# speedinghzl/CCNet

Hardware: NVIDIA H100
Metric: cca_fwd_bwd_pixels_per_s (higher is better)
Workload: dtype f32

## Files before the change

ccnet_b200/csrc/cca_tc_bwd.cuh:

```cuda
#pragma once
#include "cca_items.cuh"
#include "cca_tc_common.cuh"

namespace cca {
namespace tc {

struct BwdParams {
    ItemSpace sp;
    int C, Cq;
    long npix;
    const float *lse;
    float *delta;
    unsigned int *ddone;
    int delta_mode;
    int out_mode;
    unsigned int *cdone;
    int lag;
    int hints;
};

template <int LK, typename E> struct BwdSmem {
    using T = Tiles<LK, E>;
    static constexpr int kCh = T::H16 ? kNC : kNC / 2;
    static constexpr int kRSlot = T::kTile;
    static constexpr int off_qk = 0;
    static constexpr int off_p = off_qk + 2 * T::kSlot;
    static constexpr int off_ld = (off_p + T::kP + (16 - LK / 8) * T::kPlane + 1023) / 1024 * 1024;
    static constexpr int kTail = (128 - LK) * 128 + 256;
    static constexpr int kDsum = 1024;
    static constexpr int kBudget = 232448;
    static constexpr int kNLd = (kBudget - off_ld - kTail - kDsum - 16) / (kRSlot + 16);
    static constexpr int off_tail = off_ld + kNLd * kRSlot;
    static constexpr int off_dsum = off_tail + kTail;
    static constexpr int off_bar = off_dsum + kDsum;
    static constexpr int kBytes = off_bar + 8 * (2 + 2 * kNLd);
    static_assert(kNLd >= 8, "ring depth: chunk n - 1's dO (staged dV) up to chunk n + 1's O");
    static_assert(off_p % 1024 == 0 && T::kP >= T::kSlot, "dK staging in the P / dS planes");
    static_assert(kBytes <= kBudget, "shared memory budget");
};

__device__ __forceinline__ bool calc_delta(const BwdParams &p, const Item &it) { return p.delta_mode == 0 || (it.col && it.ik == 0); }

template <int LK, typename E>
__global__ void __launch_bounds__(kThreads, 1)
cca_tc_bwd_kernel(const __grid_constant__ CUtensorMap mqc, const __grid_constant__ CUtensorMap mqr,
                  const __grid_constant__ CUtensorMap mkc, const __grid_constant__ CUtensorMap mkr,
                  const __grid_constant__ CUtensorMap mvc, const __grid_constant__ CUtensorMap mvr,
                  const __grid_constant__ CUtensorMap mdoc, const __grid_constant__ CUtensorMap mdor,
                  const __grid_constant__ CUtensorMap moc, const __grid_constant__ CUtensorMap mor,
                  const __grid_constant__ CUtensorMap mdqc, const __grid_constant__ CUtensorMap mdqr,
                  const __grid_constant__ CUtensorMap mdkc, const __grid_constant__ CUtensorMap mdkr,
                  const __grid_constant__ CUtensorMap mdvc, const __grid_constant__ CUtensorMap mdvr, BwdParams p)
{
    using T = Tiles<LK, E>;
    using S = BwdSmem<LK, E>;
    constexpr bool H16 = kH16<E>, F16 = kF16<E>;
    constexpr int TERMS = H16 ? 1 : 3;
    constexpr int kNLd = S::kNLd;
    constexpr int kCh = S::kCh;
    constexpr int KP = LK / 16;
    constexpr uint32_t LOP = T::kPP * T::kPlane;
    extern __shared__ __align__(1024) uint8_t smem[];
    uint64_t *bars = reinterpret_cast<uint64_t *>(smem + S::off_bar);
    uint64_t *qk_full = bars, *qk_empty = bars + 1, *full = bars + 2, *empty = bars + 2 + kNLd;
    float *dsum = reinterpret_cast<float *>(smem + S::off_dsum);
    const int tid = threadIdx.x, warp = tid >> 5, lane = tid & 31;
    const int NCH = p.C / kCh;
    const int KQ = p.Cq / 16;
    const int nk = p.sp.total > (int)blockIdx.x ? (p.sp.total - (int)blockIdx.x + (int)gridDim.x - 1) / (int)gridDim.x : 0;
    auto item_of = [&](int k) { return decode_item_order(p.sp, (int)blockIdx.x + k * (int)gridDim.x, p.lag); };

    if (tid == 0) {
        mbar_init(qk_full, 1); mbar_init(qk_empty, 1);
        for (int i = 0; i < kNLd; ++i) { mbar_init(&full[i], 1); mbar_init(&empty[i], 1); }
        fence_mbar_init();
        prefetch_tmap(&mqc); prefetch_tmap(&mqr); prefetch_tmap(&mkc); prefetch_tmap(&mkr); prefetch_tmap(&mvc); prefetch_tmap(&mvr);
        prefetch_tmap(&mdoc); prefetch_tmap(&mdor); prefetch_tmap(&moc); prefetch_tmap(&mor);
        prefetch_tmap(&mdqc); prefetch_tmap(&mdqr); prefetch_tmap(&mdkc); prefetch_tmap(&mdkr); prefetch_tmap(&mdvc); prefetch_tmap(&mdvr);
    }
    __syncthreads();

    if (tid < 128) {
        setmaxnreg_dec<kProducerRegs>();
        if (warp == 0 && lane == 0) {
            const uint64_t pol_keep = l2_policy_evict_last(), pol_stream = l2_policy_evict_first();
            auto load = [&](uint8_t *dst, uint64_t *bar, const CUtensorMap *m, int c0, const Item &it, int start, bool last_use, int boxes) {
                const int cw = it.col ? it.line : start, ch = it.col ? start : it.line;
                if (p.hints == 1) {
                    const uint64_t pol = (is_producer(it) && !last_use) ? pol_keep : pol_stream;
                    for (int bx = 0; bx < boxes; ++bx) tma_load_4d(dst + bx * T::kTile, m, bar, c0 + 32 * bx, cw, ch, it.b, pol);
                } else {
                    for (int bx = 0; bx < boxes; ++bx) tma_load_4d(dst + bx * T::kTile, m, bar, c0 + 32 * bx, cw, ch, it.b);
                }
            };
            uint32_t g = 0;
            auto ring = [&](const CUtensorMap *m, int c0, const Item &it, int start, bool last_use) {
                const int slot = g % kNLd;
                mbar_wait(&empty[slot], ((g / kNLd) & 1) ^ 1);
                mbar_expect_tx(&full[slot], S::kRSlot);
                load(smem + S::off_ld + slot * S::kRSlot, &full[slot], m, c0, it, start, last_use, 1);
                ++g;
            };
            for (int k = 0; k < nk; ++k) {
                const Item it = item_of(k);
                const bool calc = calc_delta(p, it);
                mbar_wait(qk_empty, (k & 1) ^ 1);
                mbar_expect_tx(qk_full, 2 * T::kSlot);
                load(smem + S::off_qk, qk_full, it.col ? &mqc : &mqr, 0, it, it.q0, false, H16 ? 1 : 2);
                load(smem + S::off_qk + T::kSlot, qk_full, it.col ? &mkc : &mkr, 0, it, it.k0, false, H16 ? 1 : 2);
                for (int n = 0; n < NCH; ++n) {
                    ring(it.col ? &mvc : &mvr, n * kCh, it, it.k0, false);
                    ring(it.col ? &mdoc : &mdor, n * kCh, it, it.q0, false);
                    if (calc) ring(it.col ? &moc : &mor, n * kCh, it, it.q0, p.delta_mode == 1);
                }
            }
        }
    } else {
        setmaxnreg_inc<kConsumerRegs>();
        const int t = tid - 128, wg = t >> 7, wq = (t >> 5) & 3;
        const int rbase = 64 * wg + 16 * wq + (lane >> 2);
        const int cq = 2 * (lane & 3);
        const uint32_t qb = smem_u32(smem + S::off_qk), kb = qb + T::kSlot, ld_base = smem_u32(smem + S::off_ld);
        const uint32_t pb = smem_u32(smem + S::off_p);
        uint8_t *pgen = smem + S::off_p;
        const uint64_t pol_keep = l2_policy_evict_last(), pol_stream = l2_policy_evict_first();
        auto stage = [&](const float *acc, int nc, uint8_t *tile) {
#pragma unroll
            for (int h = 0; h < 2; ++h) {
                const int r = rbase + 8 * h;
                if (r >= LK) continue;
                uint8_t *row = tile + r * 128;
#pragma unroll
                for (int j = 0; j < 8; ++j) {
                    if (8 * j >= nc) break;
                    const int c = 8 * j + cq;
                    const int bx = H16 ? 0 : c >> 5, byte = H16 ? 2 * c : 4 * (c & 31);
                    uint8_t *dst = row + bx * T::kTile + ((((byte >> 4) ^ r) & 7) << 4) + (byte & 15);
                    if constexpr (H16) *reinterpret_cast<uint32_t *>(dst) = pack2<F16>(acc[4 * j + 2 * h], acc[4 * j + 2 * h + 1]);
                    else *reinterpret_cast<float2 *>(dst) = make_float2(acc[4 * j + 2 * h], acc[4 * j + 2 * h + 1]);
                }
            }
        };
        auto put = [&](const CUtensorMap *m, const uint8_t *tile, int boxes, int c0, int px0, const Item &it, bool prod) {
            const int cw = it.col ? it.line : px0, ch = it.col ? px0 : it.line;
            for (int bx = 0; bx < boxes; ++bx) {
                const uint8_t *src = tile + bx * T::kTile;
                if (p.hints == 1) {
                    if (prod) tma_store_4d(m, src, c0 + 32 * bx, cw, ch, it.b, pol_keep);
                    else tma_reduce_add_4d(m, src, c0 + 32 * bx, cw, ch, it.b, pol_stream);
                } else {
                    if (prod) tma_store_4d(m, src, c0 + 32 * bx, cw, ch, it.b);
                    else tma_reduce_add_4d(m, src, c0 + 32 * bx, cw, ch, it.b);
                }
            }
            bulk_commit();
        };
        const int qboxes = H16 ? 1 : (p.Cq > 32 ? 2 : 1);
        pdl_wait();
        uint32_t g = 0;
        int pending = -1;
        for (int k = 0; k < nk; ++k) {
            const Item it = item_of(k);
            const bool calc = calc_delta(p, it);
            const bool prod = p.out_mode == 1 && is_producer(it);
            long qpix[2];
            bool qok[2];
            float nlse[2];
            int self[2];
#pragma unroll
            for (int h = 0; h < 2; ++h) {
                const int r = rbase + 8 * h;
                qok[h] = r < it.lq;
                qpix[h] = item_pixel(p.sp, it, qok[h] ? r : 0);
                nlse[h] = qok[h] ? -p.lse[qpix[h]] * kLog2e : 0.f;
                self[h] = it.col ? it.q0 + r - it.k0 : -1;
            }
            mbar_wait(qk_full, k & 1);
            if constexpr (!H16) {
                convert_slot<LK, E>(smem + S::off_qk, t);
                convert_slot<LK, E>(smem + S::off_qk + T::kSlot, t);
            }
            {
                float acc[LK / 2];
                wg_fence();
                for (int ks = 0; ks < KQ; ++ks) {
                    wgmma_ss<LK, F16>(acc, desc_kmaj<LK, E>(qb, 64 * wg, ks, false), desc_kmaj<LK, E>(kb, 0, ks, false), ks > 0, 0, 0);
                    if constexpr (TERMS == 3) {
                        wgmma_ss<LK, F16>(acc, desc_kmaj<LK, E>(qb, 64 * wg, ks, false), desc_kmaj<LK, E>(kb, 0, ks, true), 1, 0, 0);
                        wgmma_ss<LK, F16>(acc, desc_kmaj<LK, E>(qb, 64 * wg, ks, true), desc_kmaj<LK, E>(kb, 0, ks, false), 1, 0, 0);
                    }
                }
                wg_commit();
                wg_wait<0>();
                wg_acc_fence<LK / 2>(acc);
                if (t == 0) bulk_wait_read<0>();
                consumers_sync();
#pragma unroll
                for (int j = 0; j < LK / 8; ++j)
#pragma unroll
                    for (int h = 0; h < 2; ++h) {
                        const int r = rbase + 8 * h, c = 8 * j + cq;
                        const bool ok0 = qok[h] && c < it.lk && c != self[h];
                        const bool ok1 = qok[h] && c + 1 < it.lk && c + 1 != self[h];
                        const float p0 = ok0 ? exp2f(fmaf(acc[4 * j + 2 * h], kLog2e, nlse[h])) : 0.f;
                        const float p1 = ok1 ? exp2f(fmaf(acc[4 * j + 2 * h + 1], kLog2e, nlse[h])) : 0.f;
                        if (r < LK) {
                            uint8_t *d = pgen + j * T::kPlane + r * 16 + cq * 2;
                            if constexpr (H16) {
                                *reinterpret_cast<uint32_t *>(d) = pack2<F16>(p0, p1);
                            } else {
                                uint32_t hi, lo;
                                split2(p0, p1, hi, lo);
                                *reinterpret_cast<uint32_t *>(d) = hi;
                                *reinterpret_cast<uint32_t *>(d + LOP) = lo;
                            }
                        }
                    }
            }
            fence_proxy_async();
            consumers_sync();
            if (!prod && p.out_mode == 1) wait_count(p.cdone + it.b, (unsigned)p.sp.seg0);
            if (!prod && t == 0) fence_proxy_async_global();
            float dp[LK / 2];
            float o[kCh / 2];
            float dacc = 0.f;
            const uint32_t per = calc ? 3 : 2;
            auto rslot = [&](uint32_t gi) { return gi % kNLd; };
            auto convert_chunk = [&](int n) {
                const uint32_t gv = g + per * n, gd = gv + 1, go = gv + 2;
                mbar_wait(&full[rslot(gv)], (gv / kNLd) & 1);
                mbar_wait(&full[rslot(gd)], (gd / kNLd) & 1);
                if (calc) mbar_wait(&full[rslot(go)], (go / kNLd) & 1);
                uint8_t *vs = smem + S::off_ld + rslot(gv) * S::kRSlot, *ds = smem + S::off_ld + rslot(gd) * S::kRSlot;
                if constexpr (!H16) convert_slot<LK, E, 1>(vs, t);
                if (calc) {
                    dacc += convert_slot<LK, E, 1>(ds, t, smem + S::off_ld + rslot(go) * S::kRSlot);
                    if constexpr (H16) consumers_sync();
                    if (t == 0) mbar_arrive(&empty[rslot(go)]);
                } else if constexpr (!H16) {
                    convert_slot<LK, E, 1>(ds, t);
                }
            };
            auto issue = [&](int n) {
                const uint32_t gv = g + per * n, gd = gv + 1;
                const uint32_t vb = ld_base + rslot(gv) * S::kRSlot, db = ld_base + rslot(gd) * S::kRSlot;
                wg_fence();
#pragma unroll
                for (int ks = 0; ks < kCh / 16; ++ks) {
                    wgmma_ss<LK, F16>(dp, desc_kmaj<LK, E>(db, 64 * wg, ks, false), desc_kmaj<LK, E>(vb, 0, ks, false), n > 0 || ks > 0, 0, 0);
                    if constexpr (TERMS == 3) {
                        wgmma_ss<LK, F16>(dp, desc_kmaj<LK, E>(db, 64 * wg, ks, false), desc_kmaj<LK, E>(vb, 0, ks, true), 1, 0, 0);
                        wgmma_ss<LK, F16>(dp, desc_kmaj<LK, E>(db, 64 * wg, ks, true), desc_kmaj<LK, E>(vb, 0, ks, false), 1, 0, 0);
                    }
                }
#pragma unroll
                for (int ks = 0; ks < KP; ++ks) {
                    const uint32_t pa = pb + 8 * wg * T::kPlane + ks * 256;
                    if constexpr (H16) {
                        wgmma_ss_n64<F16>(o, smem_desc(pa, 128, T::kPlane), desc_mnmaj<LK, E>(db, ks, false), ks > 0, 1, 1);
                    } else {
                        wgmma_ss_n32<1, 1>(o, smem_desc(pa, 128, T::kPlane), desc_mnmaj<LK, E>(db, ks, false), ks > 0);
                        wgmma_ss_n32<1, 1>(o, smem_desc(pa, 128, T::kPlane), desc_mnmaj<LK, E>(db, ks, true), 1);
                        wgmma_ss_n32<1, 1>(o, smem_desc(pa + LOP, 128, T::kPlane), desc_mnmaj<LK, E>(db, ks, false), 1);
                    }
                }
                wg_commit();
            };
            auto release = [&]() {
                if (t == 0 && pending >= 0) {
                    bulk_wait_read<0>();
                    mbar_arrive(&empty[pending]);
                    pending = -1;
                }
            };
            auto retire = [&](int n) {
                const uint32_t gv = g + per * n, gd = gv + 1;
                wg_acc_fence<kCh / 2>(o);
                consumers_sync();
                if (t == 0) mbar_arrive(&empty[rslot(gv)]);
                uint8_t *ds = smem + S::off_ld + rslot(gd) * S::kRSlot;
                stage(o, kCh, ds);
                fence_proxy_async();
                consumers_sync();
                if (t == 0) {
                    put(it.col ? &mdvc : &mdvr, ds, 1, n * kCh, it.k0, it, prod);
                    pending = (int)rslot(gd);
                }
            };
            convert_chunk(0);
            issue(0);
            for (int n = 0; n < NCH; ++n) {
                if (n + 1 < NCH) convert_chunk(n + 1);
                release();
                wg_wait<0>();
                retire(n);
                if (n + 1 < NCH) issue(n + 1);
            }
            wg_wait<0>();
            wg_acc_fence<LK / 2>(dp);
            g += per * NCH;
            float dl[2] = {0.f, 0.f};
            if (calc) {
                dsum[(t >> 7) * 128 + (t & 127)] = dacc;
                consumers_sync();
#pragma unroll
                for (int h = 0; h < 2; ++h) {
                    const int r = rbase + 8 * h;
                    dl[h] = dsum[r] + dsum[128 + r];
                    if (qok[h] && is_producer(it) && (lane & 3) == 0) p.delta[qpix[h]] = dl[h];
                }
                if (p.delta_mode == 1) {
                    __threadfence();
                    consumers_sync();
                    if (t == 0) atomicAdd(p.ddone + it.b, 1u);
                }
            } else {
                wait_count(p.ddone + it.b, (unsigned)p.sp.seg0);
#pragma unroll
                for (int h = 0; h < 2; ++h) dl[h] = qok[h] ? __ldcg(p.delta + qpix[h]) : 0.f;
            }
            consumers_sync();
#pragma unroll
            for (int j = 0; j < LK / 8; ++j)
#pragma unroll
                for (int h = 0; h < 2; ++h) {
                    const int r = rbase + 8 * h;
                    if (r < LK) {
                        uint8_t *d = pgen + j * T::kPlane + r * 16 + cq * 2;
                        const uint32_t hw = *reinterpret_cast<const uint32_t *>(d);
                        const uint32_t lw = H16 ? 0u : *reinterpret_cast<const uint32_t *>(d + LOP);
                        const float p0 = lo2<F16>(hw) + lo2<F16>(lw), p1 = hi2<F16>(hw) + hi2<F16>(lw);
                        const float s0 = qok[h] ? p0 * (dp[4 * j + 2 * h] - dl[h]) : 0.f;
                        const float s1 = qok[h] ? p1 * (dp[4 * j + 2 * h + 1] - dl[h]) : 0.f;
                        if constexpr (H16) {
                            *reinterpret_cast<uint32_t *>(d) = pack2<F16>(s0, s1);
                        } else {
                            uint32_t hi, lo;
                            split2(s0, s1, hi, lo);
                            *reinterpret_cast<uint32_t *>(d) = hi;
                            *reinterpret_cast<uint32_t *>(d + LOP) = lo;
                        }
                    }
                }
            fence_proxy_async();
            consumers_sync();
            {
                float aq[32], ak[32];
                wg_fence();
#pragma unroll
                for (int ks = 0; ks < KP; ++ks) {
                    const uint32_t a = pb + 64 * wg * 16 + ks * 2 * T::kPlane;
                    wgmma_ss_n64<F16>(aq, smem_desc(a, T::kPlane, 128), desc_mnmaj<LK, E>(kb, ks, false), ks > 0, 0, 1);
                    if constexpr (TERMS == 3) {
                        wgmma_ss_n64<F16>(aq, smem_desc(a, T::kPlane, 128), desc_mnmaj<LK, E>(kb, ks, true), 1, 0, 1);
                        wgmma_ss_n64<F16>(aq, smem_desc(a + LOP, T::kPlane, 128), desc_mnmaj<LK, E>(kb, ks, false), 1, 0, 1);
                    }
                }
                wg_commit();
                wg_wait<0>();
                wg_acc_fence<32>(aq);
                consumers_sync();
                stage(aq, 64, smem + S::off_qk + T::kSlot);
                fence_proxy_async();
                consumers_sync();
                if (t == 0) put(it.col ? &mdqc : &mdqr, smem + S::off_qk + T::kSlot, qboxes, 0, it.q0, it, prod);
                wg_fence();
#pragma unroll
                for (int ks = 0; ks < KP; ++ks) {
                    const uint32_t at = pb + 8 * wg * T::kPlane + ks * 256;
                    wgmma_ss_n64<F16>(ak, smem_desc(at, 128, T::kPlane), desc_mnmaj<LK, E>(qb, ks, false), ks > 0, 1, 1);
                    if constexpr (TERMS == 3) {
                        wgmma_ss_n64<F16>(ak, smem_desc(at, 128, T::kPlane), desc_mnmaj<LK, E>(qb, ks, true), 1, 1, 1);
                        wgmma_ss_n64<F16>(ak, smem_desc(at + LOP, 128, T::kPlane), desc_mnmaj<LK, E>(qb, ks, false), 1, 1, 1);
                    }
                }
                wg_commit();
                wg_wait<0>();
                wg_acc_fence<32>(ak);
                consumers_sync();
                stage(ak, 64, pgen);
                fence_proxy_async();
                consumers_sync();
                if (t == 0) {
                    put(it.col ? &mdkc : &mdkr, pgen, qboxes, 0, it.k0, it, prod);
                    bulk_wait_read<1>();
                    if (pending >= 0) mbar_arrive(&empty[pending]);
                    pending = -1;
                    mbar_arrive(qk_empty);
                    if (prod) {
                        bulk_wait<0>();
                        publish_count(p.cdone + it.b);
                    }
                }
            }
        }
        if (t == 0) bulk_wait<0>();
    }
}

namespace {
__global__ void __launch_bounds__(256) cca_bwd_prep_kernel(uint4 *dq, uint4 *dk, uint4 *dv, long nq16, long nv16,
                                                           unsigned int *counters, int n_counters)
{
    pdl_launch_dependents();
    const long tid = (long)blockIdx.x * blockDim.x + threadIdx.x, nth = (long)gridDim.x * blockDim.x;
    const uint4 z = make_uint4(0, 0, 0, 0);
    for (long i = tid; i < nq16; i += nth) { dq[i] = z; dk[i] = z; }
    for (long i = tid; i < nv16; i += nth) dv[i] = z;
    for (long i = tid; i < n_counters; i += nth) counters[i] = 0u;
}
}

template <int LK, typename E>
cudaError_t launch_bwd(const void *dout, const void *q, const void *k, const void *v, const void *out, const float *lse, float *delta,
                       unsigned int *counters, void *dq, void *dk, void *dv, Dims d, int delta_mode, cudaStream_t st,
                       const char **why)
{
    CUtensorMap m[16];
    const void *base[8] = {q, k, v, dout, out, dq, dk, dv};
    const int ch[8] = {d.Cq, d.Cq, d.C, d.C, d.C, d.Cq, d.Cq, d.C};
    BwdParams p;
    p.sp = make_space(d.B, d.H, d.W);
    for (int t = 0; t < 8; ++t)
        for (int r = 0; r < 2; ++r) {
            const int box = t < 5 ? LK : (r == 0 ? p.sp.col.tl : p.sp.row.tl);
            if (!get_map(&m[2 * t + r], base[t], d.B, d.H, d.W, ch[t], box, r == 0, kDtype<E>)) {
                if (why) *why = "cuTensorMapEncodeTiled failed";
                return cudaErrorInvalidValue;
            }
        }
    p.C = d.C; p.Cq = d.Cq;
    p.npix = (long)d.B * d.H * d.W;
    p.lse = lse; p.delta = delta;
    p.ddone = counters; p.cdone = counters + d.B;
    p.delta_mode = delta_mode;
    const bool one_tile = p.sp.col.nt == 1 && p.sp.row.nt == 1;
    p.out_mode = one_tile ? 1 : 0;
    p.lag = tc_lag() != 0 ? 1 : 0;
    p.hints = tc_l2_hints();
    const long es = sizeof(E);
    const long nq = p.out_mode == 1 ? 0 : p.npix * d.Cq * es, nv = p.out_mode == 1 ? 0 : p.npix * d.C * es;
    cca_bwd_prep_kernel<<<p.out_mode == 1 ? 1 : sm_count(), 256, 0, st>>>(
        reinterpret_cast<uint4 *>(dq), reinterpret_cast<uint4 *>(dk), reinterpret_cast<uint4 *>(dv), nq / 16, nv / 16, counters, 3 * d.B);
    count_launch();
    cudaError_t e = cudaGetLastError();
    if (e != cudaSuccess) return e;
    auto kern = cca_tc_bwd_kernel<LK, E>;
    e = cudaFuncSetAttribute(kern, cudaFuncAttributeMaxDynamicSharedMemorySize, BwdSmem<LK, E>::kBytes);
    if (e != cudaSuccess) return e;
    const int sms = sm_count();
    const int grid = p.sp.total < sms ? p.sp.total : sms;
    cudaLaunchConfig_t cfg = {};
    cfg.gridDim = dim3(grid); cfg.blockDim = dim3(kThreads); cfg.dynamicSmemBytes = BwdSmem<LK, E>::kBytes; cfg.stream = st;
    cudaLaunchAttribute attr[1];
    attr[0].id = cudaLaunchAttributeProgrammaticStreamSerialization;
    attr[0].val.programmaticStreamSerializationAllowed = 1;
    cfg.attrs = attr;
    cfg.numAttrs = tc_pdl() ? 1 : 0;
    e = cudaLaunchKernelEx(&cfg, kern, m[0], m[1], m[2], m[3], m[4], m[5], m[6], m[7], m[8], m[9], m[10], m[11], m[12], m[13],
                           m[14], m[15], p);
    count_launch();
    return e != cudaSuccess ? e : cudaGetLastError();
}


extern template cudaError_t launch_bwd<80, __half>(const void *, const void *, const void *, const void *, const void *, const float *,
                                                   float *, unsigned int *, void *, void *, void *, Dims, int, cudaStream_t,
                                                   const char **);
extern template cudaError_t launch_bwd<112, __half>(const void *, const void *, const void *, const void *, const void *, const float *,
                                                    float *, unsigned int *, void *, void *, void *, Dims, int, cudaStream_t,
                                                    const char **);

}
}
```

ccnet_b200/csrc/cca_tc_common.cuh:

```cuda
#pragma once
#include <mutex>
#include <type_traits>

#include "cca_common.cuh"
#include "cca_sm90.cuh"

namespace cca {
namespace tc {
using namespace sm90;

constexpr int kNC = 64;

constexpr int kThreads = 384;
constexpr int kConsumers = 256;
constexpr int kBarConsumers = 1;
constexpr int kBarConvert = 2;
constexpr int kProducerRegs = 40;
constexpr int kConsumerRegs = 232;
static_assert(128 * kProducerRegs + kConsumers * kConsumerRegs <= kThreads * 168, "register split exceeds the launch allocation");

template <typename E> constexpr bool kH16 = sizeof(E) == 2;
template <typename E> constexpr bool kF16 = std::is_same<E, __half>::value;
template <typename E> constexpr int kDtype = kF16<E> ? CCA_F16 : (kH16<E> ? CCA_BF16 : CCA_F32);
template <int LK, typename E> struct Tiles {
    static constexpr bool H16 = kH16<E>;
    static constexpr int kTile = LK * 128;
    static constexpr int kSlot = H16 ? kTile : 2 * kTile;
    static constexpr int kPlane = LK * 16;
    static constexpr int kPStride = 2 * kPlane;
    static constexpr int kLoOff = kPlane;
    static constexpr int kTerms = H16 ? 1 : 2;
    static constexpr int kOp = kTerms * 8 * kPlane;
    static constexpr int kPP = LK / 8;
    static constexpr int kP = kTerms * kPP * kPlane;
};

__device__ __forceinline__ uint32_t pack_bf16(float a, float b)
{
    uint32_t r;
    asm("cvt.rn.bf16x2.f32 %0, %1, %2;" : "=r"(r) : "f"(b), "f"(a));
    return r;
}
__device__ __forceinline__ void split2(float a, float b, uint32_t &hi, uint32_t &lo)
{
    hi = pack_bf16(a, b);
    const float ah = __uint_as_float(hi << 16), bh = __uint_as_float(hi & 0xFFFF0000u);
    lo = pack_bf16(a - ah, b - bh);
}
__device__ __forceinline__ void split8(const float *v, uint4 &hi, uint4 &lo)
{
    split2(v[0], v[1], hi.x, lo.x); split2(v[2], v[3], hi.y, lo.y);
    split2(v[4], v[5], hi.z, lo.z); split2(v[6], v[7], hi.w, lo.w);
}
__device__ __forceinline__ float bf_lo(uint32_t w) { return __uint_as_float(w << 16); }
__device__ __forceinline__ float bf_hi(uint32_t w) { return __uint_as_float(w & 0xFFFF0000u); }
template <bool F16> __device__ __forceinline__ uint32_t pack2(float a, float b)
{
    if constexpr (F16) {
        uint32_t r;
        asm("cvt.rn.f16x2.f32 %0, %1, %2;" : "=r"(r) : "f"(b), "f"(a));
        return r;
    } else {
        return pack_bf16(a, b);
    }
}
template <bool F16> __device__ __forceinline__ float lo2(uint32_t w)
{
    if constexpr (F16) return __half2float(__ushort_as_half((unsigned short)(w & 0xFFFFu)));
    else return bf_lo(w);
}
template <bool F16> __device__ __forceinline__ float hi2(uint32_t w)
{
    if constexpr (F16) return __half2float(__ushort_as_half((unsigned short)(w >> 16)));
    else return bf_hi(w);
}

__device__ __forceinline__ void named_bar_sync(int id, int nthreads)
{
    asm volatile("bar.sync %0, %1;" ::"r"(id), "r"(nthreads) : "memory");
}
__device__ __forceinline__ void consumers_sync() { named_bar_sync(kBarConsumers, kConsumers); }

template <int LK, typename E, int NB = 2>
__device__ __forceinline__ float convert_slot(uint8_t *slot, int t, const uint8_t *dot = nullptr)
{
    using T = Tiles<LK, E>;
    constexpr bool H16 = T::H16, F16 = kF16<E>;
    const int r = t & 127, hq = t >> 7;
    const int rr = r < LK ? r : LK - 1, sw = rr & 7;
    float acc = 0.f;
    if constexpr (H16) {
        if (dot) {
#pragma unroll
            for (int j = 0; j < 4; ++j) {
                const int c = (hq * 4 + j) ^ sw;
                const uint4 x = *reinterpret_cast<const uint4 *>(slot + rr * 128 + c * 16);
                const uint4 y = *reinterpret_cast<const uint4 *>(dot + rr * 128 + c * 16);
                const uint32_t xw[4] = {x.x, x.y, x.z, x.w}, yw[4] = {y.x, y.y, y.z, y.w};
#pragma unroll
                for (int e = 0; e < 4; ++e) acc += lo2<F16>(xw[e]) * lo2<F16>(yw[e]) + hi2<F16>(xw[e]) * hi2<F16>(yw[e]);
            }
        }
        return r < LK ? acc : 0.f;
    } else {
        static_assert(NB == 1 || NB == 2, "boxes per slot");
        float4 raw[4 * NB];
#pragma unroll
        for (int bx = 0; bx < NB; ++bx)
#pragma unroll
            for (int j = 0; j < 4; ++j)
                raw[4 * bx + j] = *reinterpret_cast<const float4 *>(slot + bx * T::kTile + rr * 128 + (((hq * 4 + j) ^ sw) * 16));
        if (dot) {
#pragma unroll
            for (int bx = 0; bx < NB; ++bx)
#pragma unroll
                for (int j = 0; j < 4; ++j) {
                    const float4 o = *reinterpret_cast<const float4 *>(dot + bx * T::kTile + rr * 128 + (((hq * 4 + j) ^ sw) * 16));
                    const float4 x = raw[4 * bx + j];
                    acc += x.x * o.x + x.y * o.y + x.z * o.z + x.w * o.w;
                }
        }
        named_bar_sync(kBarConvert, kConsumers);
        if (r < LK) {
#pragma unroll
            for (int bx = 0; bx < NB; ++bx) {
                uint8_t *d = slot + bx * T::kTile + r * 16 + hq * 2 * T::kPStride;
#pragma unroll
                for (int j = 0; j < 2; ++j) {
                    const float4 a = raw[4 * bx + 2 * j], b = raw[4 * bx + 2 * j + 1];
                    const float v[8] = {a.x, a.y, a.z, a.w, b.x, b.y, b.z, b.w};
                    uint4 hi, lo;
                    split8(v, hi, lo);
                    *reinterpret_cast<uint4 *>(d + j * T::kPStride) = hi;
                    *reinterpret_cast<uint4 *>(d + j * T::kPStride + T::kLoOff) = lo;
                }
            }
        }
        fence_proxy_async();
        consumers_sync();
        return r < LK ? acc : 0.f;
    }
}

template <int LK, typename E> __device__ __forceinline__ uint64_t desc_kmaj(uint32_t slot, int row0, int ks, bool lo)
{
    using T = Tiles<LK, E>;
    if constexpr (T::H16) return smem_desc(slot + row0 * 128 + ks * 32, 16, 1024, kSw128);
    else return smem_desc(slot + row0 * 16 + ks * 2 * T::kPStride + (lo ? T::kLoOff : 0), T::kPStride, 128);
}
template <int LK, typename E> __device__ __forceinline__ uint64_t desc_mnmaj(uint32_t slot, int ks, bool lo)
{
    using T = Tiles<LK, E>;
    if constexpr (T::H16) return smem_desc(slot + ks * 2048, 16, 1024, kSw128);
    else return smem_desc(slot + ks * 256 + (lo ? T::kLoOff : 0), 128, T::kPStride);
}

typedef CUresult (*EncodeFn)(CUtensorMap *, CUtensorMapDataType, cuuint32_t, void *, const cuuint64_t *, const cuuint64_t *,
                             const cuuint32_t *, const cuuint32_t *, CUtensorMapInterleave, CUtensorMapSwizzle,
                             CUtensorMapL2promotion, CUtensorMapFloatOOBfill);
inline EncodeFn get_encode()
{
    static EncodeFn fn = nullptr;
    static std::once_flag once;
    std::call_once(once, [] {
        cudaDriverEntryPointQueryResult qr;
        void *p = nullptr;
        if (cudaGetDriverEntryPoint("cuTensorMapEncodeTiled", &p, cudaEnableDefault, &qr) == cudaSuccess &&
            qr == cudaDriverEntryPointSuccess)
            fn = reinterpret_cast<EncodeFn>(p);
    });
    return fn;
}
inline bool make_map(CUtensorMap *m, const void *base, int B, int H, int W, int C, int LK, bool col, int dtype)
{
    EncodeFn enc = get_encode();
    if (!enc) return false;
    const bool h16 = dtype != CCA_F32;
    const cuuint64_t es_bytes = h16 ? 2 : 4;
    cuuint64_t dims[4] = {(cuuint64_t)C, (cuuint64_t)W, (cuuint64_t)H, (cuuint64_t)B};
    cuuint64_t strides[3] = {(cuuint64_t)C * es_bytes, (cuuint64_t)W * C * es_bytes, (cuuint64_t)H * W * C * es_bytes};
    cuuint32_t box[4] = {h16 ? 64u : 32u, col ? 1u : (cuuint32_t)LK, col ? (cuuint32_t)LK : 1u, 1};
    cuuint32_t es[4] = {1, 1, 1, 1};
    const CUtensorMapDataType et = dtype == CCA_F16    ? CU_TENSOR_MAP_DATA_TYPE_FLOAT16
                                   : dtype == CCA_BF16 ? CU_TENSOR_MAP_DATA_TYPE_BFLOAT16
                                                       : CU_TENSOR_MAP_DATA_TYPE_FLOAT32;
    return enc(m, et, 4, const_cast<void *>(base), dims, strides, box, es,
               CU_TENSOR_MAP_INTERLEAVE_NONE, CU_TENSOR_MAP_SWIZZLE_128B, CU_TENSOR_MAP_L2_PROMOTION_L2_256B,
               CU_TENSOR_MAP_FLOAT_OOB_FILL_NONE) == CUDA_SUCCESS;
}
inline int lk_for(int tile) { return tile <= 80 ? 80 : (tile <= 112 ? 112 : 0); }
bool get_map(CUtensorMap *m, const void *base, int B, int H, int W, int C, int LK, bool col, int dtype);
int sm_count();
inline bool shape_supported(Dims d, int dtype)
{
    if (dtype != CCA_F32 && dtype != CCA_BF16 && dtype != CCA_F16) return false;
    if (d.Cq % 16 != 0 || d.Cq > 64 || d.Cq < 16 || d.C % kNC != 0) return false;
    if (d.H > 112 * 8 || d.W > 112 * 8) return false;
    return get_encode() != nullptr;
}

}
}
```

Baseline: 36.43 million.

## Split Q/K barriers, prefetch next LSE, and defer dependency publish in backward

```diff
diff --git a/ccnet_b200/csrc/cca_tc_bwd.cuh b/ccnet_b200/csrc/cca_tc_bwd.cuh
--- a/ccnet_b200/csrc/cca_tc_bwd.cuh
+++ b/ccnet_b200/csrc/cca_tc_bwd.cuh
@@ -29,11 +29,11 @@
     static constexpr int kTail = (128 - LK) * 128 + 256;
     static constexpr int kDsum = 1024;
     static constexpr int kBudget = 232448;
-    static constexpr int kNLd = (kBudget - off_ld - kTail - kDsum - 16) / (kRSlot + 16);
+    static constexpr int kNLd = (kBudget - off_ld - kTail - kDsum - 32) / (kRSlot + 16);
     static constexpr int off_tail = off_ld + kNLd * kRSlot;
     static constexpr int off_dsum = off_tail + kTail;
     static constexpr int off_bar = off_dsum + kDsum;
-    static constexpr int kBytes = off_bar + 8 * (2 + 2 * kNLd);
+    static constexpr int kBytes = off_bar + 8 * (4 + 2 * kNLd);
     static_assert(kNLd >= 8, "ring depth: chunk n - 1's dO (staged dV) up to chunk n + 1's O");
     static_assert(off_p % 1024 == 0 && T::kP >= T::kSlot, "dK staging in the P / dS planes");
     static_assert(kBytes <= kBudget, "shared memory budget");
@@ -62,7 +62,7 @@
     constexpr uint32_t LOP = T::kPP * T::kPlane;
     extern __shared__ __align__(1024) uint8_t smem[];
     uint64_t *bars = reinterpret_cast<uint64_t *>(smem + S::off_bar);
-    uint64_t *qk_full = bars, *qk_empty = bars + 1, *full = bars + 2, *empty = bars + 2 + kNLd;
+    uint64_t *q_full = bars, *k_full = bars + 1, *q_empty = bars + 2, *k_empty = bars + 3, *full = bars + 4, *empty = bars + 4 + kNLd;
     float *dsum = reinterpret_cast<float *>(smem + S::off_dsum);
     const int tid = threadIdx.x, warp = tid >> 5, lane = tid & 31;
     const int NCH = p.C / kCh;
@@ -71,7 +71,7 @@
     auto item_of = [&](int k) { return decode_item_order(p.sp, (int)blockIdx.x + k * (int)gridDim.x, p.lag); };
 
     if (tid == 0) {
-        mbar_init(qk_full, 1); mbar_init(qk_empty, 1);
+        mbar_init(q_full, 1); mbar_init(k_full, 1); mbar_init(q_empty, 1); mbar_init(k_empty, 1);
         for (int i = 0; i < kNLd; ++i) { mbar_init(&full[i], 1); mbar_init(&empty[i], 1); }
         fence_mbar_init();
         prefetch_tmap(&mqc); prefetch_tmap(&mqr); prefetch_tmap(&mkc); prefetch_tmap(&mkr); prefetch_tmap(&mvc); prefetch_tmap(&mvr);
@@ -104,10 +104,12 @@
             for (int k = 0; k < nk; ++k) {
                 const Item it = item_of(k);
                 const bool calc = calc_delta(p, it);
-                mbar_wait(qk_empty, (k & 1) ^ 1);
-                mbar_expect_tx(qk_full, 2 * T::kSlot);
-                load(smem + S::off_qk, qk_full, it.col ? &mqc : &mqr, 0, it, it.q0, false, H16 ? 1 : 2);
-                load(smem + S::off_qk + T::kSlot, qk_full, it.col ? &mkc : &mkr, 0, it, it.k0, false, H16 ? 1 : 2);
+                mbar_wait(k_empty, (k & 1) ^ 1);
+                mbar_expect_tx(k_full, T::kSlot);
+                load(smem + S::off_qk + T::kSlot, k_full, it.col ? &mkc : &mkr, 0, it, it.k0, false, H16 ? 1 : 2);
+                mbar_wait(q_empty, (k & 1) ^ 1);
+                mbar_expect_tx(q_full, T::kSlot);
+                load(smem + S::off_qk, q_full, it.col ? &mqc : &mqr, 0, it, it.q0, false, H16 ? 1 : 2);
                 for (int n = 0; n < NCH; ++n) {
                     ring(it.col ? &mvc : &mvr, n * kCh, it, it.k0, false);
                     ring(it.col ? &mdoc : &mdor, n * kCh, it, it.q0, false);
@@ -159,6 +161,16 @@
         pdl_wait();
         uint32_t g = 0;
         int pending = -1;
+        int publish = -1;
+        float lse_row[2] = {0.f, 0.f};
+        auto load_lse = [&](const Item &nx) {
+#pragma unroll
+            for (int h = 0; h < 2; ++h) {
+                const int r = rbase + 8 * h;
+                if (r < nx.lq) lse_row[h] = p.lse[item_pixel(p.sp, nx, r)];
+            }
+        };
+        if (nk > 0) load_lse(item_of(0));
         for (int k = 0; k < nk; ++k) {
             const Item it = item_of(k);
             const bool calc = calc_delta(p, it);
@@ -172,14 +184,13 @@
                 const int r = rbase + 8 * h;
                 qok[h] = r < it.lq;
                 qpix[h] = item_pixel(p.sp, it, qok[h] ? r : 0);
-                nlse[h] = qok[h] ? -p.lse[qpix[h]] * kLog2e : 0.f;
+                nlse[h] = qok[h] ? -lse_row[h] * kLog2e : 0.f;
                 self[h] = it.col ? it.q0 + r - it.k0 : -1;
             }
-            mbar_wait(qk_full, k & 1);
-            if constexpr (!H16) {
-                convert_slot<LK, E>(smem + S::off_qk, t);
-                convert_slot<LK, E>(smem + S::off_qk + T::kSlot, t);
-            }
+            mbar_wait(k_full, k & 1);
+            if constexpr (!H16) convert_slot<LK, E>(smem + S::off_qk + T::kSlot, t);
+            mbar_wait(q_full, k & 1);
+            if constexpr (!H16) convert_slot<LK, E>(smem + S::off_qk, t);
             {
                 float acc[LK / 2];
                 wg_fence();
@@ -191,6 +202,11 @@
                     }
                 }
                 wg_commit();
+                if (t == 0 && publish >= 0) {
+                    bulk_wait<0>();
+                    publish_count(p.cdone + publish);
+                    publish = -1;
+                }
                 wg_wait<0>();
                 wg_acc_fence<LK / 2>(acc);
                 if (t == 0) bulk_wait_read<0>();
@@ -298,6 +314,7 @@
             }
             wg_wait<0>();
             wg_acc_fence<LK / 2>(dp);
+            if (k + 1 < nk) load_lse(item_of(k + 1));
             g += per * NCH;
             float dl[2] = {0.f, 0.f};
             if (calc) {
@@ -375,26 +392,29 @@
                     }
                 }
                 wg_commit();
+                if (t == 0) {
+                    bulk_wait_read<0>();
+                    if (pending >= 0) mbar_arrive(&empty[pending]);
+                    pending = -1;
+                    mbar_arrive(k_empty);
+                }
                 wg_wait<0>();
                 wg_acc_fence<32>(ak);
                 consumers_sync();
+                if (t == 0) mbar_arrive(q_empty);
                 stage(ak, 64, pgen);
                 fence_proxy_async();
                 consumers_sync();
                 if (t == 0) {
                     put(it.col ? &mdkc : &mdkr, pgen, qboxes, 0, it.k0, it, prod);
-                    bulk_wait_read<1>();
-                    if (pending >= 0) mbar_arrive(&empty[pending]);
-                    pending = -1;
-                    mbar_arrive(qk_empty);
-                    if (prod) {
-                        bulk_wait<0>();
-                        publish_count(p.cdone + it.b);
-                    }
+                    if (prod) publish = it.b;
                 }
             }
         }
-        if (t == 0) bulk_wait<0>();
+        if (t == 0) {
+            bulk_wait<0>();
+            if (publish >= 0) publish_count(p.cdone + publish);
+        }
     }
 }
 
```

New measurement: 36.70 million, median of 6. About the same (+0.8%).

## Stream Q/K through load ring and overlap dP with dV staging

Applied to the files above, without the earlier changes.

```diff
diff --git a/ccnet_b200/csrc/cca_tc_bwd.cuh b/ccnet_b200/csrc/cca_tc_bwd.cuh
--- a/ccnet_b200/csrc/cca_tc_bwd.cuh
+++ b/ccnet_b200/csrc/cca_tc_bwd.cuh
@@ -29,11 +29,11 @@
     static constexpr int kTail = (128 - LK) * 128 + 256;
     static constexpr int kDsum = 1024;
     static constexpr int kBudget = 232448;
-    static constexpr int kNLd = (kBudget - off_ld - kTail - kDsum - 16) / (kRSlot + 16);
+    static constexpr int kNLd = (kBudget - off_ld - kTail - kDsum) / (kRSlot + 16);
     static constexpr int off_tail = off_ld + kNLd * kRSlot;
     static constexpr int off_dsum = off_tail + kTail;
     static constexpr int off_bar = off_dsum + kDsum;
-    static constexpr int kBytes = off_bar + 8 * (2 + 2 * kNLd);
+    static constexpr int kBytes = off_bar + 8 * 2 * kNLd;
     static_assert(kNLd >= 8, "ring depth: chunk n - 1's dO (staged dV) up to chunk n + 1's O");
     static_assert(off_p % 1024 == 0 && T::kP >= T::kSlot, "dK staging in the P / dS planes");
     static_assert(kBytes <= kBudget, "shared memory budget");
@@ -59,10 +59,11 @@
     constexpr int kNLd = S::kNLd;
     constexpr int kCh = S::kCh;
     constexpr int KP = LK / 16;
+    constexpr int kQKBoxes = H16 ? 1 : 2;
     constexpr uint32_t LOP = T::kPP * T::kPlane;
     extern __shared__ __align__(1024) uint8_t smem[];
     uint64_t *bars = reinterpret_cast<uint64_t *>(smem + S::off_bar);
-    uint64_t *qk_full = bars, *qk_empty = bars + 1, *full = bars + 2, *empty = bars + 2 + kNLd;
+    uint64_t *full = bars, *empty = bars + kNLd;
     float *dsum = reinterpret_cast<float *>(smem + S::off_dsum);
     const int tid = threadIdx.x, warp = tid >> 5, lane = tid & 31;
     const int NCH = p.C / kCh;
@@ -71,7 +72,6 @@
     auto item_of = [&](int k) { return decode_item_order(p.sp, (int)blockIdx.x + k * (int)gridDim.x, p.lag); };
 
     if (tid == 0) {
-        mbar_init(qk_full, 1); mbar_init(qk_empty, 1);
         for (int i = 0; i < kNLd; ++i) { mbar_init(&full[i], 1); mbar_init(&empty[i], 1); }
         fence_mbar_init();
         prefetch_tmap(&mqc); prefetch_tmap(&mqr); prefetch_tmap(&mkc); prefetch_tmap(&mkr); prefetch_tmap(&mvc); prefetch_tmap(&mvr);
@@ -84,30 +84,26 @@
         setmaxnreg_dec<kProducerRegs>();
         if (warp == 0 && lane == 0) {
             const uint64_t pol_keep = l2_policy_evict_last(), pol_stream = l2_policy_evict_first();
-            auto load = [&](uint8_t *dst, uint64_t *bar, const CUtensorMap *m, int c0, const Item &it, int start, bool last_use, int boxes) {
-                const int cw = it.col ? it.line : start, ch = it.col ? start : it.line;
-                if (p.hints == 1) {
-                    const uint64_t pol = (is_producer(it) && !last_use) ? pol_keep : pol_stream;
-                    for (int bx = 0; bx < boxes; ++bx) tma_load_4d(dst + bx * T::kTile, m, bar, c0 + 32 * bx, cw, ch, it.b, pol);
-                } else {
-                    for (int bx = 0; bx < boxes; ++bx) tma_load_4d(dst + bx * T::kTile, m, bar, c0 + 32 * bx, cw, ch, it.b);
-                }
-            };
             uint32_t g = 0;
             auto ring = [&](const CUtensorMap *m, int c0, const Item &it, int start, bool last_use) {
                 const int slot = g % kNLd;
                 mbar_wait(&empty[slot], ((g / kNLd) & 1) ^ 1);
                 mbar_expect_tx(&full[slot], S::kRSlot);
-                load(smem + S::off_ld + slot * S::kRSlot, &full[slot], m, c0, it, start, last_use, 1);
+                uint8_t *dst = smem + S::off_ld + slot * S::kRSlot;
+                const int cw = it.col ? it.line : start, ch = it.col ? start : it.line;
+                if (p.hints == 1) {
+                    const uint64_t pol = (is_producer(it) && !last_use) ? pol_keep : pol_stream;
+                    tma_load_4d(dst, m, &full[slot], c0, cw, ch, it.b, pol);
+                } else {
+                    tma_load_4d(dst, m, &full[slot], c0, cw, ch, it.b);
+                }
                 ++g;
             };
             for (int k = 0; k < nk; ++k) {
                 const Item it = item_of(k);
                 const bool calc = calc_delta(p, it);
-                mbar_wait(qk_empty, (k & 1) ^ 1);
-                mbar_expect_tx(qk_full, 2 * T::kSlot);
-                load(smem + S::off_qk, qk_full, it.col ? &mqc : &mqr, 0, it, it.q0, false, H16 ? 1 : 2);
-                load(smem + S::off_qk + T::kSlot, qk_full, it.col ? &mkc : &mkr, 0, it, it.k0, false, H16 ? 1 : 2);
+                for (int bx = 0; bx < kQKBoxes; ++bx) ring(it.col ? &mqc : &mqr, 32 * bx, it, it.q0, false);
+                for (int bx = 0; bx < kQKBoxes; ++bx) ring(it.col ? &mkc : &mkr, 32 * bx, it, it.k0, false);
                 for (int n = 0; n < NCH; ++n) {
                     ring(it.col ? &mvc : &mvr, n * kCh, it, it.k0, false);
                     ring(it.col ? &mdoc : &mdor, n * kCh, it, it.q0, false);
@@ -159,6 +155,7 @@
         pdl_wait();
         uint32_t g = 0;
         int pending = -1;
+        int unpublished = -1;
         for (int k = 0; k < nk; ++k) {
             const Item it = item_of(k);
             const bool calc = calc_delta(p, it);
@@ -175,10 +172,36 @@
                 nlse[h] = qok[h] ? -p.lse[qpix[h]] * kLog2e : 0.f;
                 self[h] = it.col ? it.q0 + r - it.k0 : -1;
             }
-            mbar_wait(qk_full, k & 1);
-            if constexpr (!H16) {
-                convert_slot<LK, E>(smem + S::off_qk, t);
-                convert_slot<LK, E>(smem + S::off_qk + T::kSlot, t);
+            {
+                const uint8_t *src[2 * kQKBoxes];
+#pragma unroll
+                for (int i = 0; i < 2 * kQKBoxes; ++i) {
+                    const uint32_t gi = g + i;
+                    mbar_wait(&full[gi % kNLd], (gi / kNLd) & 1);
+                    src[i] = smem + S::off_ld + (gi % kNLd) * S::kRSlot;
+                }
+                if constexpr (H16) {
+                    constexpr int kV = T::kTile / 16, kPer = (kV + kConsumers - 1) / kConsumers;
+                    uint4 v[2][kPer];
+#pragma unroll
+                    for (int i = 0; i < 2; ++i)
+#pragma unroll
+                        for (int j = 0; j < kPer; ++j)
+                            if (t + kConsumers * j < kV) v[i][j] = reinterpret_cast<const uint4 *>(src[i])[t + kConsumers * j];
+                    consumers_sync();
+#pragma unroll
+                    for (int i = 0; i < 2; ++i)
+#pragma unroll
+                        for (int j = 0; j < kPer; ++j)
+                            if (t + kConsumers * j < kV) reinterpret_cast<uint4 *>(smem + S::off_qk + i * T::kSlot)[t + kConsumers * j] = v[i][j];
+                    fence_proxy_async();
+                    consumers_sync();
+                } else {
+                    convert_slot<LK, E, 4>(smem + S::off_qk, t, nullptr, src);
+                }
+                if (t == 0)
+                    for (int i = 0; i < 2 * kQKBoxes; ++i) mbar_arrive(&empty[(g + i) % kNLd]);
+                g += 2 * kQKBoxes;
             }
             {
                 float acc[LK / 2];
@@ -193,7 +216,15 @@
                 wg_commit();
                 wg_wait<0>();
                 wg_acc_fence<LK / 2>(acc);
-                if (t == 0) bulk_wait_read<0>();
+                if (t == 0) {
+                    if (unpublished >= 0) {
+                        bulk_wait<0>();
+                        publish_count(p.cdone + unpublished);
+                        unpublished = -1;
+                    } else {
+                        bulk_wait_read<0>();
+                    }
+                }
                 consumers_sync();
 #pragma unroll
                 for (int j = 0; j < LK / 8; ++j)
@@ -219,8 +250,6 @@
             }
             fence_proxy_async();
             consumers_sync();
-            if (!prod && p.out_mode == 1) wait_count(p.cdone + it.b, (unsigned)p.sp.seg0);
-            if (!prod && t == 0) fence_proxy_async_global();
             float dp[LK / 2];
             float o[kCh / 2];
             float dacc = 0.f;
@@ -232,16 +261,53 @@
                 mbar_wait(&full[rslot(gd)], (gd / kNLd) & 1);
                 if (calc) mbar_wait(&full[rslot(go)], (go / kNLd) & 1);
                 uint8_t *vs = smem + S::off_ld + rslot(gv) * S::kRSlot, *ds = smem + S::off_ld + rslot(gd) * S::kRSlot;
-                if constexpr (!H16) convert_slot<LK, E, 1>(vs, t);
-                if (calc) {
-                    dacc += convert_slot<LK, E, 1>(ds, t, smem + S::off_ld + rslot(go) * S::kRSlot);
-                    if constexpr (H16) consumers_sync();
-                    if (t == 0) mbar_arrive(&empty[rslot(go)]);
-                } else if constexpr (!H16) {
-                    convert_slot<LK, E, 1>(ds, t);
+                const uint8_t *os = smem + S::off_ld + rslot(go) * S::kRSlot;
+                if constexpr (H16) {
+                    if (calc) {
+                        dacc += convert_slot<LK, E, 1>(ds, t, os);
+                        consumers_sync();
+                        if (t == 0) mbar_arrive(&empty[rslot(go)]);
+                    }
+                } else {
+                    const int r = t & 127, hq = t >> 7;
+                    const int rr = r < LK ? r : LK - 1, sw = rr & 7;
+                    float4 raw[2][4];
+#pragma unroll
+                    for (int j = 0; j < 4; ++j) {
+                        raw[0][j] = *reinterpret_cast<const float4 *>(vs + rr * 128 + (((hq * 4 + j) ^ sw) * 16));
+                        raw[1][j] = *reinterpret_cast<const float4 *>(ds + rr * 128 + (((hq * 4 + j) ^ sw) * 16));
+                    }
+                    if (calc) {
+                        float acc = 0.f;
+#pragma unroll
+                        for (int j = 0; j < 4; ++j) {
+                            const float4 o = *reinterpret_cast<const float4 *>(os + rr * 128 + (((hq * 4 + j) ^ sw) * 16));
+                            const float4 x = raw[1][j];
+                            acc += x.x * o.x + x.y * o.y + x.z * o.z + x.w * o.w;
+                        }
+                        dacc += r < LK ? acc : 0.f;
+                    }
+                    named_bar_sync(kBarConvert, kConsumers);
+                    if (calc && t == 0) mbar_arrive(&empty[rslot(go)]);
+                    if (r < LK) {
+#pragma unroll
+                        for (int b = 0; b < 2; ++b) {
+                            uint8_t *d = (b ? ds : vs) + r * 16 + hq * 2 * T::kPStride;
+#pragma unroll
+                            for (int j = 0; j < 2; ++j) {
+                                const float4 a = raw[b][2 * j], c = raw[b][2 * j + 1];
+                                const float v[8] = {a.x, a.y, a.z, a.w, c.x, c.y, c.z, c.w};
+                                uint4 hi, lo;
+                                split8(v, hi, lo);
+                                *reinterpret_cast<uint4 *>(d + j * T::kPStride) = hi;
+                                *reinterpret_cast<uint4 *>(d + j * T::kPStride + T::kLoOff) = lo;
+                            }
+                        }
+                    }
+                    fence_proxy_async();
                 }
             };
-            auto issue = [&](int n) {
+            auto issue_dp = [&](int n) {
                 const uint32_t gv = g + per * n, gd = gv + 1;
                 const uint32_t vb = ld_base + rslot(gv) * S::kRSlot, db = ld_base + rslot(gd) * S::kRSlot;
                 wg_fence();
@@ -253,6 +319,11 @@
                         wgmma_ss<LK, F16>(dp, desc_kmaj<LK, E>(db, 64 * wg, ks, true), desc_kmaj<LK, E>(vb, 0, ks, false), 1, 0, 0);
                     }
                 }
+                wg_commit();
+            };
+            auto issue_dv = [&](int n) {
+                const uint32_t db = ld_base + rslot(g + per * n + 1) * S::kRSlot;
+                wg_fence();
 #pragma unroll
                 for (int ks = 0; ks < KP; ++ks) {
                     const uint32_t pa = pb + 8 * wg * T::kPlane + ks * 256;
@@ -273,28 +344,31 @@
                     pending = -1;
                 }
             };
-            auto retire = [&](int n) {
-                const uint32_t gv = g + per * n, gd = gv + 1;
-                wg_acc_fence<kCh / 2>(o);
-                consumers_sync();
-                if (t == 0) mbar_arrive(&empty[rslot(gv)]);
-                uint8_t *ds = smem + S::off_ld + rslot(gd) * S::kRSlot;
-                stage(o, kCh, ds);
-                fence_proxy_async();
-                consumers_sync();
-                if (t == 0) {
-                    put(it.col ? &mdvc : &mdvr, ds, 1, n * kCh, it.k0, it, prod);
-                    pending = (int)rslot(gd);
-                }
-            };
             convert_chunk(0);
-            issue(0);
+            if constexpr (!H16) consumers_sync();
+            issue_dp(0);
+            issue_dv(0);
             for (int n = 0; n < NCH; ++n) {
                 if (n + 1 < NCH) convert_chunk(n + 1);
                 release();
                 wg_wait<0>();
-                retire(n);
-                if (n + 1 < NCH) issue(n + 1);
+                wg_acc_fence<kCh / 2>(o);
+                if (n == 0 && !prod) {
+                    if (p.out_mode == 1) wait_count(p.cdone + it.b, (unsigned)p.sp.seg0);
+                    if (t == 0) fence_proxy_async_global();
+                }
+                consumers_sync();
+                if (t == 0) mbar_arrive(&empty[rslot(g + per * n)]);
+                if (n + 1 < NCH) issue_dp(n + 1);
+                uint8_t *ds = smem + S::off_ld + rslot(g + per * n + 1) * S::kRSlot;
+                stage(o, kCh, ds);
+                fence_proxy_async();
+                consumers_sync();
+                if (t == 0) {
+                    put(it.col ? &mdvc : &mdvr, ds, 1, n * kCh, it.k0, it, prod);
+                    pending = (int)rslot(g + per * n + 1);
+                }
+                if (n + 1 < NCH) issue_dv(n + 1);
             }
             wg_wait<0>();
             wg_acc_fence<LK / 2>(dp);
@@ -386,15 +460,14 @@
                     bulk_wait_read<1>();
                     if (pending >= 0) mbar_arrive(&empty[pending]);
                     pending = -1;
-                    mbar_arrive(qk_empty);
-                    if (prod) {
-                        bulk_wait<0>();
-                        publish_count(p.cdone + it.b);
-                    }
+                    if (prod) unpublished = it.b;
                 }
             }
         }
-        if (t == 0) bulk_wait<0>();
+        if (t == 0) {
+            bulk_wait<0>();
+            if (unpublished >= 0) publish_count(p.cdone + unpublished);
+        }
     }
 }
 
diff --git a/ccnet_b200/csrc/cca_tc_common.cuh b/ccnet_b200/csrc/cca_tc_common.cuh
--- a/ccnet_b200/csrc/cca_tc_common.cuh
+++ b/ccnet_b200/csrc/cca_tc_common.cuh
@@ -82,7 +82,7 @@
 __device__ __forceinline__ void consumers_sync() { named_bar_sync(kBarConsumers, kConsumers); }
 
 template <int LK, typename E, int NB = 2>
-__device__ __forceinline__ float convert_slot(uint8_t *slot, int t, const uint8_t *dot = nullptr)
+__device__ __forceinline__ float convert_slot(uint8_t *slot, int t, const uint8_t *dot = nullptr, const uint8_t *const *src = nullptr)
 {
     using T = Tiles<LK, E>;
     constexpr bool H16 = T::H16, F16 = kF16<E>;
@@ -103,13 +103,13 @@
         }
         return r < LK ? acc : 0.f;
     } else {
-        static_assert(NB == 1 || NB == 2, "boxes per slot");
+        static_assert(NB == 1 || NB == 2 || NB == 4, "boxes per slot");
         float4 raw[4 * NB];
 #pragma unroll
         for (int bx = 0; bx < NB; ++bx)
 #pragma unroll
             for (int j = 0; j < 4; ++j)
-                raw[4 * bx + j] = *reinterpret_cast<const float4 *>(slot + bx * T::kTile + rr * 128 + (((hq * 4 + j) ^ sw) * 16));
+                raw[4 * bx + j] = *reinterpret_cast<const float4 *>((src ? src[bx] : slot + bx * T::kTile) + rr * 128 + (((hq * 4 + j) ^ sw) * 16));
         if (dot) {
 #pragma unroll
             for (int bx = 0; bx < NB; ++bx)
```

Measured after the change: 36.90 million before, 38.12 million after (median of 6 runs). 3.3% higher.
